# ZackAttack614/BlackBird

Hardware: AMD Instinct MI355X
Metric: selfplay_games_per_sec (higher is better)
Workload: dtype f32 (float32 operands split exactly into 3 bf16 values, 6 bf16 MFMA products each, f32 accumulate)

## Files before the change

### blackbird_amd/csrc/tree.hip.h

```cpp
#pragma once
#include "games.hip.h"
#include "rng.hip.h"
#include "starts.h"
#include "stamps.hip.h"

#define NODE_EXPANDED 1
#define NODE_TERMINAL 2
#define NODE_CACHED 4
#define LEAF_RECORDED 0x40000000
#define CHILD_NONE (-1)
#define CHILD_TERM_BIT 0x40000000

template <class G>
struct alignas(128) DenseNode {
    int32_t flags;
    uint32_t legal_mask;
    int32_t all;
    int32_t serial;
    double sq;
    double pad0;
    int32_t N[G::S];
    float Q[G::S];
    int32_t child[G::S];
    alignas(128) double cP[G::S];
    float W[G::S];
    typename G::State st;
};

struct ExampleHdr {
    uint32_t game_id;
    uint16_t ply;
    uint8_t player;
    int8_t z;
    uint32_t total;
    uint32_t n_children;
};

#define BB_SLOTS_TREE(B, Q, R)                                                                     \
    B(int32_t, root, 1) B(int32_t, root_N, 1) B(int32_t, n_nodes, 1) B(int32_t, ply, 1) B(int32_t, sims_left, 1)           \
    B(int32_t, pend_leaf, 1) B(int32_t, pend_expand, 1) B(int32_t, path_len, 1)                                            \
    B(int32_t, game_lid, 1)                                             \
    B(int32_t, sim_serial, 1) B(float, root_W, 1)                                                                          \
    B(int8_t, root_pp, 1)                                   \
    B(uint32_t, path, MP)                                                                \
        \
    R(int32_t, path_N, MP) R(int32_t, path_all, MP)       \
    R(float, path_W, MP)                                                               \
    Q(int32_t, leaf_flags, 1)
#define BB_SLOTS_ANC(X)                                                                                 \
       \
    X(uint32_t, anc, ANC)                                                                                                   \
    X(int32_t, anc_len, 1) X(int32_t, top_N, 1)
#define BB_SLOTS_MAILBOX(B, Q)                                                 \
    B(uint32_t, leaf_game_id, 1) B(int32_t, leaf_serial, 1) B(float, eval_value, 1) Q(float, eval_policy, PS)              \
    B(uint64_t, evals, 1)                                                              \
    B(uint64_t, ctr, 8)
#define BB_SLOTS_OUT(X)                                                       \
    X(int32_t, out_action, 1) X(int32_t, out_root_plays, 1) X(int32_t, out_child_plays, S)                                 \
    X(float, out_root_winrate, 1) X(float, out_child_value, S)
#define BB_SLOTS_RESUME(X) X(int32_t, resume_cur, 1) X(int32_t, resume_depth, 1)
#define BB_SLOTS_POST(X) X(int, post_slot, 1)
#define BB_ROW_NONE(...)
#define BB_SLOT_ARRAYS(X) BB_SLOTS_TREE(X, X, X) BB_SLOTS_ANC(X) BB_SLOTS_MAILBOX(X, X) BB_SLOTS_OUT(X) BB_SLOTS_RESUME(X) BB_SLOTS_POST(X)
#define BB_SLOT_SHADOWED(X) BB_SLOTS_TREE(X, BB_ROW_NONE, BB_ROW_NONE) BB_SLOTS_MAILBOX(X, BB_ROW_NONE)
#define BB_SLOT_POINTER(T, f, per) T *f;
#define BB_SHADOW_MEMBER(T, f, per) T f[GW * (per)];
#define BB_SHADOW_LOAD(o, f, per) for (int i = threadIdx.x; i < n * (per); i += nthreads) f[i] = o.f[(size_t)g0 * (per) + i];
#define BB_SHADOW_STORE(o, f, per) for (int i = threadIdx.x; i < n * (per); i += nthreads) o.f[(size_t)g0 * (per) + i] = f[i];

struct TreeDev {
    int n_slots, node_cap, sims_per_move, max_plies, kind, max_depth, evaluator, priors_ones;
    int salt_per_game, max_games;
    int gpw;
    double c_puct;
    uint64_t seed, salt;
    uint32_t first_game_id;
    BB_SLOTS_TREE(BB_SLOT_POINTER, BB_SLOT_POINTER, BB_SLOT_POINTER)
    int track_anc;
    BB_SLOTS_ANC(BB_SLOT_POINTER)
    void *leaf_state;
    BB_SLOTS_MAILBOX(BB_SLOT_POINTER, BB_SLOT_POINTER)
    void *nodes;
    int n_games_target;
    double temp;
    uint8_t *examples;
    int32_t *game_hdr;
    int example_bytes;
    BB_SLOTS_OUT(BB_SLOT_POINTER)
    const double *in_u;
    BB_SLOTS_RESUME(BB_SLOT_POINTER)
    int *post_count;
    BB_SLOTS_POST(BB_SLOT_POINTER)
    int level_budget;
    int slot_offset;
    int lid_stride;
    int pool_g0;
    int *visit_pool;
    float noise_alpha;
    void *eval_cache;
    int eval_cache_log2;
    unsigned long long *eval_cache_ctr;
    unsigned long long *stamps;
    const void *starts;
    int n_starts;
    double temp_late;
    int temp_plies;
};

template <int STEP>
__device__ __forceinline__ int dpp_step_i(int v) {
    if (STEP == 0) return __builtin_amdgcn_update_dpp(v, v, 0xB1, 0xf, 0xf, false);
    if (STEP == 1) return __builtin_amdgcn_update_dpp(v, v, 0x4E, 0xf, 0xf, false);
    if (STEP == 2) return __builtin_amdgcn_update_dpp(v, v, 0x141, 0xf, 0xf, false);
    return __builtin_amdgcn_update_dpp(v, v, 0x140, 0xf, 0xf, false);
}
template <int STEP>
__device__ __forceinline__ double dpp_step_d(double v) {
    long long b = __double_as_longlong(v);
    int lo = dpp_step_i<STEP>((int)(b & 0xffffffffll)), hi = dpp_step_i<STEP>((int)(b >> 32));
    return __longlong_as_double(((long long)hi << 32) | (unsigned int)lo);
}

template <int S>
__device__ __forceinline__ int grp_sum_i(int v) {
    v += dpp_step_i<0>(v);
    v += dpp_step_i<1>(v);
    v += dpp_step_i<2>(v);
    if (S == 16) v += dpp_step_i<3>(v);
    return v;
}

template <int A, int S>
__device__ __forceinline__ double grp_np_sum(double x) {
    double a[A];
#pragma unroll
    for (int k = 0; k < A; k++) a[k] = __shfl(x, k, S);
    if (A < 8) {
        double res = 0.;
#pragma unroll
        for (int k = 0; k < A; k++) res += a[k];
        return res;
    } else {
        double r[8];
#pragma unroll
        for (int j = 0; j < 8; j++) r[j] = a[j];
        int i = 8;
        for (; i < A - (A % 8); i += 8)
            for (int j = 0; j < 8; j++) r[j] += a[i + j];
        double res = ((r[0] + r[1]) + (r[2] + r[3])) + ((r[4] + r[5]) + (r[6] + r[7]));
        for (; i < A; i++) res += a[i];
        return res;
    }
}

template <int S, int STEP>
__device__ __forceinline__ void argmax_step(double &u, int &idx, int &payload) {
    double ou = dpp_step_d<STEP>(u);
    int oi = dpp_step_i<STEP>(idx), op = dpp_step_i<STEP>(payload);
    if (ou > u || (ou == u && oi < idx)) {
        u = ou;
        idx = oi;
        payload = op;
    }
}
template <int S>
__device__ __forceinline__ int grp_argmax(double u, int idx, int &payload) {
    (void)idx;
    double m = u;
    m = __builtin_fmax(m, dpp_step_d<0>(m));
    m = __builtin_fmax(m, dpp_step_d<1>(m));
    m = __builtin_fmax(m, dpp_step_d<2>(m));
    if (S == 16) m = __builtin_fmax(m, dpp_step_d<3>(m));
    const unsigned long long eq = __ballot(u == m);
    const int l64 = (int)__lane_id();
    const unsigned grp = (unsigned)(eq >> (l64 & ~(S - 1))) & ((1u << S) - 1u);
    const int win = __ffs(grp) - 1;
    payload = __shfl(payload, win, S);
    return win;
}

__device__ __forceinline__ double puct_score(double q, double cPi, double sq, int Ni, bool legal) {
    double u = q + __ddiv_rn(cPi * sq, 1.0 + (double)Ni);
    return legal ? u : -1.0;
}
#ifndef BB_PUCT_FILTER
#define BB_PUCT_FILTER 1
#endif
template <int S>
__device__ __forceinline__ int grp_argmax_puct(float qf, double cPi, double sq, int Ni, bool legal, int &payload) {
#if BB_PUCT_FILTER
    const float num = (float)(cPi * sq);
    const float uf = legal ? __builtin_fmaf(num, __builtin_amdgcn_rcpf((float)(Ni + 1)), qf) : -1.0f;
    float mf = uf;
    mf = __builtin_fmaxf(mf, __int_as_float(dpp_step_i<0>(__float_as_int(mf))));
    mf = __builtin_fmaxf(mf, __int_as_float(dpp_step_i<1>(__float_as_int(mf))));
    mf = __builtin_fmaxf(mf, __int_as_float(dpp_step_i<2>(__float_as_int(mf))));
    if (S == 16) mf = __builtin_fmaxf(mf, __int_as_float(dpp_step_i<3>(__float_as_int(mf))));
    const bool mine = uf >= mf - mf * 0x1p-18f && uf >= 0.0f;
    const unsigned long long cand = __ballot(mine);
    const int l64 = (int)__lane_id();
    const unsigned grp = (unsigned)(cand >> (l64 & ~(S - 1))) & ((1u << S) - 1u);
    if (__ballot((grp & (grp - 1u)) != 0u || grp == 0u) == 0ull) {
        const int win = __ffs(grp) - 1;
        int p = mine ? payload : 0;
        p |= dpp_step_i<0>(p);
        p |= dpp_step_i<1>(p);
        p |= dpp_step_i<2>(p);
        if (S == 16) p |= dpp_step_i<3>(p);
        payload = p;
        return win;
    }
#endif
    return grp_argmax<S>(puct_score((double)qf, cPi, sq, Ni, legal), 0, payload);
}
__device__ __forceinline__ double child_q(const TreeDev &d, float Qi, float Wi, int Ni) {
    if (d.evaluator != 2) return (double)Qi;
    return Ni > 0 ? (double)Wi / (double)Ni : 0.0;
}

__device__ __forceinline__ uint32_t path_word(int node, int player, int a) {
    return ((uint32_t)node << 6) | ((uint32_t)player << 4) | (uint32_t)a;
}
#define ANC_BROKEN (-1)

template <class G, bool REC = false>
__device__ __forceinline__ void backup_path(const TreeDev &d, int g, int lane, DenseNode<G> *pool, int plen, float v01,
                                            int prev) {
    constexpr int S = G::S;
    const float vflip = 1.0f - v01;
    const size_t p0 = (size_t)g * G::MAXPATH;
    auto edge = [&](uint32_t e, int k) __attribute__((always_inline)) {
        const int a = e & 15, pl = (e >> 4) & 3;
        DenseNode<G> *pn = pool + (e >> 6);
        int n, all;
        float w;
        if constexpr (REC) { n = d.path_N[p0 + k]; all = d.path_all[p0 + k]; w = d.path_W[p0 + k]; }
        else { n = pn->N[a]; all = pn->all; w = pn->W[a]; }
        n += 1;
        all += 1;
        w += (pl == prev) ? v01 : vflip;
        pn->N[a] = n;
        pn->W[a] = w;
        pn->Q[a] = __fdiv_rn(w, (float)n);
        pn->all = all;
        pn->sq = __dsqrt_rn(1.0 + (double)all);
    };
    for (int k = lane; k < plen; k += S) edge(d.path[p0 + k], k);
    if constexpr (!REC) {
        if (d.track_anc) {
            const uint32_t *anc = d.anc + (size_t)g * (d.max_plies + 2);
            const int na = d.anc_len[g];
            for (int k = lane; k < na; k += S) edge(anc[k], 0);
            if (lane == 0) d.top_N[g] += 1;
        }
    }
    if (lane == 0) {
        d.root_N[g] += 1;
        int pp = d.root_pp[g];
        if (pp) d.root_W[g] += (pp == prev) ? v01 : vflip;
    }
}

template <class G, bool REC = false>
__device__ __forceinline__ void phase_apply(const TreeDev &d, int g, int lane) {
    using Node = DenseNode<G>;
    constexpr int S = G::S, A = G::A;
    const int leaf = d.pend_leaf[g];
    if (leaf < 0) return;
    int lf = 0;
    if constexpr (REC) lf = d.leaf_flags[g] & ~LEAF_RECORDED;
    Node *pool = (Node *)d.nodes + (size_t)(g + d.pool_g0) * d.node_cap;
    Node *node = pool + leaf;
    auto add_flag = [&](int bit) __attribute__((always_inline)) {
        if constexpr (REC) node->flags = lf | bit;
        else node->flags |= bit;
    };
    const typename G::State st = ((const typename G::State *)d.leaf_state)[g];
    const float v = d.eval_value[g];
    const int expand_rec = REC ? d.pend_expand[g] : 0;
    auto expand = [&]() __attribute__((always_inline)) { return REC ? expand_rec : d.pend_expand[g]; };
    if (expand()) {
        const uint32_t mask = G::legal_mask(st);
        double x = 0.0;
        if (lane < A) x = (double)d.eval_policy[(size_t)g * S + lane] * (double)((mask >> lane) & 1u);
        const double tot = grp_np_sum<A, S>(x);
        node->N[lane] = 0;
        node->Q[lane] = 0.f;
        node->W[lane] = 0.f;
        node->child[lane] = CHILD_NONE;
        node->cP[lane] = (lane < A) ? d.c_puct * __ddiv_rn(x, tot) : 0.0;
        if (lane == 0) {
            add_flag(NODE_EXPANDED);
            node->legal_mask = mask;
            node->all = 0;
            node->sq = 1.0;
        }
    }
    const int player = gs_player(st), prev = gs_prev(st);
    const bool f32_eval = REC || d.evaluator != 2;
    float v01 = v;
    if (f32_eval) {
        v01 = (v + 1.0f) * 0.5f;
        if (player != prev) v01 = 1.0f - v01;
    }
    if (f32_eval && !expand() && ((REC ? lf : node->flags) & NODE_TERMINAL) && lane == 0) {
        node->pad0 = (double)v01;
        add_flag(NODE_CACHED);
    }
    backup_path<G, REC>(d, g, lane, pool, d.path_len[g], v01, prev);
    if (lane == 0) d.pend_leaf[g] = -1;
}

template <class G>
__device__ __forceinline__ int create_child(const TreeDev &d, int g, DenseNode<G> *pool, DenseNode<G> *parent,
                                            const typename G::State &pst, int a, int lane, int &nn,
                                            typename G::State &st2, bool &terminal, int *flags_out = nullptr) {
    int idx = nn;
    st2 = pst;
    G::apply(st2, a);
    int w = G::winner(st2, a);
    terminal = w >= 0;
    if (idx >= d.node_cap) return CHILD_NONE;
    int word = idx | (terminal ? CHILD_TERM_BIT : 0);
    nn = idx + 1;
    const int cflags = (terminal ? (NODE_TERMINAL | ((w + 1) << 8)) : 0) | (gs_player(st2) << 4);
    if (flags_out) *flags_out = cflags;
    if (lane == 0) {
        DenseNode<G> *c = pool + idx;
        c->st = st2;
        c->flags = cflags;
        c->legal_mask = 0;
        c->all = 0;
        c->serial = idx;
        parent->child[a] = word;
        d.n_nodes[g] = idx + 1;
        d.ctr[(size_t)g * 8 + 2] += 1;
    }
    return word;
}

template <class G>
__device__ __forceinline__ uint32_t expand_ones(const TreeDev &d, DenseNode<G> *node, const typename G::State &st,
                                                int lane, double &cPi) {
    uint32_t mask = G::legal_mask(st);
    cPi = (lane < G::A && ((mask >> lane) & 1u)) ? d.c_puct * 1.0 : 0.0;
    node->N[lane] = 0;
    node->Q[lane] = 0.f;
    node->W[lane] = 0.f;
    node->child[lane] = CHILD_NONE;
    node->cP[lane] = cPi;
    if (lane == 0) {
        node->flags |= NODE_EXPANDED;
        node->legal_mask = mask;
        node->all = 0;
        node->sq = 1.0;
    }
    return mask;
}

template <class G>
__device__ __forceinline__ void post_leaf(const TreeDev &d, int g, int cur, const typename G::State &st, int flags_word, int expand,
                                          int depth) {
    ((typename G::State *)d.leaf_state)[g] = st;
    d.leaf_game_id[g] = d.first_game_id + (uint32_t)d.game_lid[g];
    d.leaf_serial[g] = cur;
    d.pend_leaf[g] = cur;
    if (d.leaf_flags) d.leaf_flags[g] = flags_word;
    d.pend_expand[g] = expand;
    d.path_len[g] = depth;
    d.sim_serial[g] += 1;
    d.evals[g] += 1;
}

template <class G>
__device__ void phase_select(const TreeDev &d, int g, int lane) {
    using Node = DenseNode<G>;
    constexpr int S = G::S, A = G::A;
    if (d.game_lid[g] < 0 || d.sims_left[g] <= 0) return;
    Node *pool = (Node *)d.nodes + (size_t)(g + d.pool_g0) * d.node_cap;
    uint32_t *path = d.path + (size_t)g * G::MAXPATH;
    int cur = d.root[g];
    int nn = d.n_nodes[g];
    int depth = 0, expand = 0, overflow = 0, term_leaf = 0;
    const bool inline_expand = d.priors_ones != 0;
    const bool fixed = d.kind == 1, rollout = d.evaluator == 2;
    typename G::State st;
    int flags = 0;
    bool have = false;
    IF_STAMPS(long long acc_load = 0, acc_iter = 0;)
    for (int it = 0;; it++) {
        IF_STAMPS(long long ts0 = clock64(); acc_iter++;)
        Node *node = pool + cur;
        typename G::State st_l = node->st;
        int flags_l = node->flags;
        uint32_t mask = node->legal_mask;
        double sq = node->sq;
        int Ni = node->N[lane];
        float Qi = node->Q[lane];
        float Wi = rollout ? node->W[lane] : 0.f;
        double cPi = node->cP[lane];
        int ci = node->child[lane];
        asm volatile("" ::"v"(flags_l), "v"(mask), "v"(sq), "v"(Ni), "v"(Qi), "v"(cPi), "v"(ci));
        IF_STAMPS(acc_load += clock64() - ts0;)
        if (!have) {
            st = st_l;
            flags = flags_l;
        }
        have = false;
        if (fixed && it >= d.max_depth) break;
        if (!(flags & NODE_EXPANDED)) {
            if (flags & NODE_TERMINAL) { term_leaf = 1; break; }
            if (!inline_expand) { expand = 1; break; }
            mask = expand_ones<G>(d, node, st, lane, cPi);
            if (!fixed) break;
            Ni = 0;
            Qi = 0.f;
            Wi = 0.f;
            sq = 1.0;
            ci = CHILD_NONE;
        }
        if (mask == 0) break;
        double u = puct_score(child_q(d, Qi, Wi, Ni), cPi, sq, Ni, lane < A && ((mask >> lane) & 1u));
        int child = ci;
        int a = grp_argmax<S>(u, lane, child);
        if (depth >= G::MAXPATH) { overflow = 1; break; }
        if (child == CHILD_NONE) {
            typename G::State st2;
            bool terminal;
            child = create_child<G>(d, g, pool, node, st, a, lane, nn, st2, terminal);
            if (child == CHILD_NONE) { overflow = 1; break; }
            if (lane == 0) path[depth] = path_word(cur, (flags >> 4) & 3, a);
            st = st2;
            flags = (terminal ? NODE_TERMINAL : 0) | (gs_player(st2) << 4);
            have = true;
        } else {
            if (lane == 0) path[depth] = path_word(cur, (flags >> 4) & 3, a);
        }
        depth++;
        cur = child & ~CHILD_TERM_BIT;
    }
    if (lane == 0) {
        IF_STAMPS(stamp_add(d.stamps, TS_ROW_LOAD, acc_load); stamp_add(d.stamps, TS_ITERATIONS, acc_iter); stamp_add(d.stamps, TS_DESCENTS, 1);)
        post_leaf<G>(d, g, cur, st, 0, expand, depth);
        d.sims_left[g] -= 1;
        uint64_t *c = d.ctr + (size_t)g * 8;
        c[0] += 1;
        c[1] += (uint64_t)depth;
        c[3] += (uint64_t)term_leaf;
        c[6] += (uint64_t)overflow;
    }
}

template <class G>
__global__ void __launch_bounds__(256) k_tree_step(TreeDev d) {
    constexpr int S = G::S;
    int t = blockIdx.x * blockDim.x + threadIdx.x;
    int wv = t >> 6, l64 = t & 63;
    if (l64 >= d.gpw * S) return;
    int g = wv * d.gpw + l64 / S, lane = l64 % S;
    if (g >= d.n_slots) return;
    const long long t0 = stamp_clock();
    phase_apply<G>(d, g, lane);
    const long long t1 = stamp_clock();
    __threadfence_block();
    const long long t2 = stamp_clock();
    phase_select<G>(d, g, lane);
    const long long t3 = stamp_clock();
    if ((threadIdx.x & 63) == 0) {
        stamp_add(d.stamps, TS_APPLY, t1 - t0);
        stamp_add(d.stamps, TS_FENCE, t2 - t1);
        stamp_add(d.stamps, TS_SELECT, t3 - t2);
        stamp_add(d.stamps, TS_WAVES, 1);
    }
}

template <class G>
__global__ void __launch_bounds__(256) k_tree_apply(TreeDev d) {
    constexpr int S = G::S;
    int t = blockIdx.x * blockDim.x + threadIdx.x;
    int g = t / S, lane = t % S;
    if (g >= d.n_slots) return;
    phase_apply<G>(d, g, lane);
}

template <class G>
__device__ __forceinline__ int choose_move(const TreeDev &d, int g, int lane, double temp, double u, int &total, int &Ni_out,
                           float &Wi_out) {
    using Node = DenseNode<G>;
    constexpr int S = G::S, A = G::A;
    Node *pool = (Node *)d.nodes + (size_t)(g + d.pool_g0) * d.node_cap;
    Node *node = pool + d.root[g];
    if (!(node->flags & NODE_EXPANDED)) {
        total = 0;
        Ni_out = 0;
        Wi_out = 0.f;
        return -3;
    }
    uint32_t mask = node->legal_mask;
    bool legal = lane < A && ((mask >> lane) & 1u);
    int Ni = legal ? node->N[lane] : 0;
    float Wi = legal ? node->W[lane] : 0.f;
    Ni_out = Ni;
    Wi_out = Wi;
    int all = grp_sum_i<S>(Ni);
    total = all;
    if (temp == 0.0) {
        double uu = puct_score(child_q(d, node->Q[lane], Wi, Ni), node->cP[lane], node->sq, Ni, legal);
        int dummy = 0;
        return grp_argmax<S>(uu, lane, dummy);
    }
    double it = 1.0 / temp;
    double w = (it == 1.0) ? (double)Ni : pow((double)Ni, it);
    double ws[A];
#pragma unroll
    for (int k = 0; k < A; k++) ws[k] = __shfl(w, k, S);
    double allp = 0.0;
#pragma unroll
    for (int k = 0; k < A; k++) allp += ws[k];
    if (!(allp > 0.0 && allp < INFINITY)) return -4;
    double last = 0.0;
#pragma unroll
    for (int k = 0; k < A; k++) last += __ddiv_rn(ws[k], allp);
    double run = 0.0;
    int act = A - 1;
    bool found = false;
#pragma unroll
    for (int k = 0; k < A; k++) {
        run += __ddiv_rn(ws[k], allp);
        if (!found && __ddiv_rn(run, last) > u) {
            act = k;
            found = true;
        }
    }
    return act;
}

template <class G>
__global__ void __launch_bounds__(256) k_sample(TreeDev d, double temp) {
    constexpr int S = G::S;
    int t = blockIdx.x * blockDim.x + threadIdx.x;
    int g = t / S, lane = t % S;
    if (g >= d.n_slots) return;
    if (d.game_lid[g] < 0) {
        if (lane == 0 && d.out_action) d.out_action[g] = -3;
        return;
    }
    double u = d.in_u ? d.in_u[g] : bb_u53(d.seed, d.first_game_id + (uint32_t)d.game_lid[g], (uint32_t)d.ply[g]);
    int total, Ni;
    float Wi;
    int act = choose_move<G>(d, g, lane, temp, u, total, Ni, Wi);
    if (d.out_child_plays) d.out_child_plays[(size_t)g * S + lane] = Ni;
    if (d.out_child_value) d.out_child_value[(size_t)g * S + lane] = Wi;
    if (lane == 0) {
        if (d.out_action) d.out_action[g] = act;
        if (d.out_root_plays) d.out_root_plays[g] = d.root_N[g];
        if (d.out_root_winrate) {
            int n = d.root_N[g];
            float w = d.root_W[g];
            d.out_root_winrate[g] = n > 0 ? ((d.evaluator == 2) ? (float)((double)w / (double)n) : __fdiv_rn(w, (float)n)) : 0.f;
        }
    }
}

template <class G, bool CHAIN = true>
__device__ __forceinline__ void advance_root(const TreeDev &d, int g, int lane, int a, typename G::State &new_st) {
    using Node = DenseNode<G>;
    Node *pool = (Node *)d.nodes + (size_t)(g + d.pool_g0) * d.node_cap;
    Node *node = pool + d.root[g];
    typename G::State st = node->st;
    if (!(node->flags & NODE_EXPANDED)) {
        new_st = st;
        G::apply(new_st, a);
        if (lane == 0) {
            Node *r = pool;
            r->st = new_st;
            r->flags = gs_player(new_st) << 4;
            r->serial = 0;
            d.n_nodes[g] = 1;
            d.root[g] = 0;
            d.root_N[g] = 0;
            d.root_W[g] = 0.f;
            d.root_pp[g] = 0;
            if (d.track_anc) {
                d.anc_len[g] = 0;
                d.top_N[g] = 0;
            }
        }
        return;
    }
    int child = node->child[a];
    int cn = node->N[a];
    float cw = node->W[a];
    if (child == CHILD_NONE) {
        bool terminal;
        int nn = d.n_nodes[g];
        child = create_child<G>(d, g, pool, node, st, a, lane, nn, new_st, terminal);
        if (child == CHILD_NONE) {
            child = 0;
            cn = 0;
            cw = 0.f;
            if (lane == 0) {
                pool->st = new_st;
                pool->flags = gs_player(new_st) << 4;
                d.n_nodes[g] = 1;
                d.ctr[(size_t)g * 8 + 6] += 1;
            }
        }
    } else {
        new_st = pool[child & ~CHILD_TERM_BIT].st;
    }
    if (lane == 0) {
        if (d.track_anc) {
            if (child == 0 && cn == 0 && d.n_nodes[g] == 1) {
                d.anc_len[g] = 0;
                d.top_N[g] = 0;
            } else if constexpr (!CHAIN) {
                if (d.anc_len[g] < d.max_plies + 2) {
                    d.anc[(size_t)g * (d.max_plies + 2) + d.anc_len[g]] = path_word(d.root[g], gs_player(st), a);
                    d.anc_len[g] += 1;
                }
            } else {
                const int na = d.anc_len[g], cap = d.max_plies + 2;
                if (na >= 0 && na < cap) {
                    d.anc[(size_t)g * cap + na] = path_word(d.root[g], gs_player(st), a);
                    d.anc_len[g] = na + 1;
                } else {
                    d.anc_len[g] = ANC_BROKEN;
                }
            }
        }
        d.root[g] = child & ~CHILD_TERM_BIT;
        d.root_N[g] = cn;
        d.root_W[g] = cw;
        d.root_pp[g] = (int8_t)gs_player(st);
    }
}

template <class G>
__global__ void __launch_bounds__(256) k_reset_roots(TreeDev d) {
    int g = blockIdx.x * blockDim.x + threadIdx.x;
    if (g >= d.n_slots || !d.track_anc || d.game_lid[g] < 0 || d.anc_len[g] <= 0) return;
    {
        const int na = d.anc_len[g];
        const bool parked = d.resume_cur[g] >= 0, posted = d.pend_leaf[g] >= 0;
        const int plen = parked ? d.resume_depth[g] : d.path_len[g];
        if (parked || posted) {
            if (plen + na <= G::MAXPATH) {
                uint32_t *path = d.path + (size_t)g * G::MAXPATH;
                const uint32_t *anc = d.anc + (size_t)g * (d.max_plies + 2);
                for (int k = plen - 1; k >= 0; k--) path[k + na] = path[k];
                for (int k = 0; k < na; k++) path[k] = anc[k];
                if (parked) d.resume_depth[g] = plen + na;
                else d.path_len[g] = plen + na;
            } else {
                d.ctr[(size_t)g * 8 + 6] += 1;
            }
        }
    }
    d.root[g] = (int)(d.anc[(size_t)g * (d.max_plies + 2)] >> 6);
    d.root_N[g] = d.top_N[g];
    d.root_W[g] = 0.f;
    d.root_pp[g] = 0;
    d.anc_len[g] = 0;
}

template <class G>
__global__ void __launch_bounds__(64) k_node_view(TreeDev d, int g, int node, int32_t *child_out, int32_t *plays_out, float *value_out,
                                                   typename G::State *state_out, int32_t *info_out) {
    using Node = DenseNode<G>;
    const int lane = threadIdx.x;
    if (lane >= G::S) return;
    Node *pool = (Node *)d.nodes + (size_t)(g + d.pool_g0) * d.node_cap;
    if (node < 0) node = d.root[g];
    const Node *n = pool + node;
    const bool exp = (n->flags & NODE_EXPANDED) != 0;
    child_out[lane] = exp ? n->child[lane] : CHILD_NONE;
    plays_out[lane] = exp ? n->N[lane] : 0;
    value_out[lane] = exp ? n->W[lane] : 0.f;
    if (lane == 0) {
        *state_out = n->st;
        info_out[0] = n->flags;
        info_out[1] = (int32_t)(exp ? n->legal_mask : 0u);
        info_out[2] = node;
    }
}

template <class G>
__global__ void __launch_bounds__(256) k_move_roots(TreeDev d, const int32_t *actions) {
    constexpr int S = G::S;
    int t = blockIdx.x * blockDim.x + threadIdx.x;
    int g = t / S, lane = t % S;
    if (g >= d.n_slots) return;
    int a = actions[g];
    if (a < 0 || a >= G::A || d.game_lid[g] < 0) return;
    typename G::State ns;
    advance_root<G>(d, g, lane, a, ns);
    if (lane == 0) d.ply[g] += 1;
}

template <class G>
__device__ __forceinline__ void reset_slot(const TreeDev &d, int g, int lid, const typename G::State &st) {
    using Node = DenseNode<G>;
    Node *pool = (Node *)d.nodes + (size_t)(g + d.pool_g0) * d.node_cap;
    pool->st = st;
    pool->flags = gs_player(st) << 4;
    pool->legal_mask = 0;
    pool->all = 0;
    pool->serial = 0;
    d.n_nodes[g] = 1;
    d.root[g] = 0;
    d.root_N[g] = 0;
    d.root_W[g] = 0.f;
    d.root_pp[g] = 0;
    d.ply[g] = 0;
    d.pend_leaf[g] = -1;
    d.pend_expand[g] = 0;
    d.path_len[g] = 0;
    d.sim_serial[g] = 0;
    d.game_lid[g] = lid;
    if (d.leaf_flags) d.leaf_flags[g] = 0;
    if (d.track_anc) {
        d.anc_len[g] = 0;
        d.top_N[g] = 0;
    }
}

template <class G>
__global__ void __launch_bounds__(256) k_set_roots(TreeDev d, int n, const int32_t *slots,
                                                   const typename G::State *states, const uint32_t *game_ids) {
    int i = blockIdx.x * blockDim.x + threadIdx.x;
    if (i >= n) return;
    int g = slots ? slots[i] : i;
    if (g < 0 || g >= d.n_slots) return;
    reset_slot<G>(d, g, game_ids ? (int)game_ids[i] : g, states[i]);
    d.sims_left[g] = 0;
}

__global__ void __launch_bounds__(256) k_add_sims(TreeDev d, int sims, const uint8_t *mask = nullptr) {
    int g = blockIdx.x * blockDim.x + threadIdx.x;
    if (g >= d.n_slots) return;
    if (d.game_lid[g] >= 0 && (!mask || mask[g])) d.sims_left[g] = sims;
}

template <class G>
__global__ void __launch_bounds__(256) k_get_roots(TreeDev d, typename G::State *out) {
    int g = blockIdx.x * blockDim.x + threadIdx.x;
    if (g >= d.n_slots) return;
    out[g] = ((DenseNode<G> *)d.nodes + (size_t)(g + d.pool_g0) * d.node_cap + d.root[g])->st;
}

template <class G>
__device__ __forceinline__ typename G::State start_state(const TreeDev &d, int lid) {
    const typename G::State *t = (const typename G::State *)d.starts;
    if (t && lid >= 0) return t[lid % d.n_starts];
    return G::initial();
}

template <class G>
__global__ void __launch_bounds__(256) k_check_starts(int n, const typename G::State *states, uint8_t *verdict) {
    int i = blockIdx.x * blockDim.x + threadIdx.x;
    if (i >= n) return;
    const typename G::State st = states[i];
    int v = BB_START_OK;
    if (G::winner(st, -1) >= 0) v = BB_START_FINISHED;
    else if (G::legal_mask(st) == 0) v = BB_START_NO_MOVE;
    verdict[i] = (uint8_t)v;
}

template <class G>
__global__ void __launch_bounds__(256) k_selfplay_begin(TreeDev d) {
    int g = blockIdx.x * blockDim.x + threadIdx.x;
    if (g >= d.n_slots) return;
    if (g + d.slot_offset < d.n_games_target) {
        reset_slot<G>(d, g, g + d.slot_offset, start_state<G>(d, g + d.slot_offset));
        d.sims_left[g] = d.sims_per_move;
    } else {
        reset_slot<G>(d, g, -1, start_state<G>(d, -1));
        d.sims_left[g] = 0;
    }
}

template <class G>
__device__ __forceinline__ uint8_t *example_ptr(const TreeDev &d, int lid, int ply) {
    return d.examples + ((size_t)lid * (d.max_plies + 1) + ply) * d.example_bytes;
}

template <class G>
__device__ __forceinline__ void write_example(const TreeDev &d, int lid, int ply, const typename G::State &st, int lane, int Ni,
                              int total, uint32_t gid) {
    uint8_t *p = example_ptr<G>(d, lid, ply);
    if (lane == 0) {
        ExampleHdr h;
        h.game_id = gid;
        h.ply = (uint16_t)ply;
        h.player = (uint8_t)gs_player(st);
        h.z = 0;
        h.total = (uint32_t)total;
        h.n_children = G::A;
        *(ExampleHdr *)p = h;
        *(typename G::State *)(p + sizeof(ExampleHdr)) = st;
    }
    ((uint32_t *)(p + sizeof(ExampleHdr) + sizeof(typename G::State)))[lane] = (uint32_t)Ni;
}

template <class G, bool CHAIN = true>
__device__ __forceinline__ void selfplay_move_body(const TreeDev &d, int g, int lane) {
    using Node = DenseNode<G>;
    constexpr int S = G::S;
    int lid = d.game_lid[g];
    if (lid < 0) return;
    Node *pool = (Node *)d.nodes + (size_t)(g + d.pool_g0) * d.node_cap;
    typename G::State st = pool[d.root[g]].st;
    uint32_t gid = d.first_game_id + (uint32_t)lid;
    int ply = d.ply[g];
    double u = bb_u53(d.seed, gid, (uint32_t)ply);
    int total, Ni;
    float Wi;
    int act = choose_move<G>(d, g, lane, ply < d.temp_plies ? d.temp : d.temp_late, u, total, Ni, Wi);
    if (act < 0) {
        if (lane == 0) {
            d.game_lid[g] = -1;
            d.ctr[(size_t)g * 8 + 6] += 1;
        }
        return;
    }
    write_example<G>(d, lid, ply, st, lane, Ni, total, gid);
    typename G::State ns;
    advance_root<G, CHAIN>(d, g, lane, act, ns);
    __threadfence_block();
    ply += 1;
    int w = G::winner(ns, -1);
    bool over = w >= 0 || ply >= d.max_plies;
    if (!over) {
        if (lane == 0) {
            d.ply[g] = ply;
            d.sims_left[g] = d.sims_per_move;
            d.ctr[(size_t)g * 8 + 5] += 1;
        }
        return;
    }
    write_example<G>(d, lid, ply, ns, lane, 0, 0, gid);
    __threadfence_block();
    for (int k = lane; k <= ply; k += S) {
        ExampleHdr *h = (ExampleHdr *)example_ptr<G>(d, lid, k);
        h->z = (w <= 0) ? 0 : (h->player == w ? 1 : -1);
    }
    __threadfence();
    if (lane == 0) {
        int32_t *gh = d.game_hdr + (size_t)lid * 4;
        gh[0] = ply + 1;
        gh[1] = w;
        gh[2] = ply;
        __threadfence();
        gh[3] = 1;
        uint64_t *c = d.ctr + (size_t)g * 8;
        c[4] += 1;
        c[5] += 1;
        c[7] += (uint64_t)(ply + 1);
        int next = lid + d.lid_stride;
        if (next < d.n_games_target) {
            reset_slot<G>(d, g, next, start_state<G>(d, next));
            d.sims_left[g] = d.sims_per_move;
        } else {
            d.game_lid[g] = -1;
            d.sims_left[g] = 0;
        }
    }
}

template <class G>
__global__ void __launch_bounds__(256) k_selfplay_move(TreeDev d) {
    constexpr int S = G::S;
    int t = blockIdx.x * blockDim.x + threadIdx.x;
    int g = t / S, lane = t % S;
    if (g >= d.n_slots) return;
    phase_apply<G>(d, g, lane);
    __threadfence_block();
    selfplay_move_body<G>(d, g, lane);
}

struct NoPostHook {
    __device__ __forceinline__ void operator()(int, int) const {}
};
template <class G, bool REC = false, class OnPost = NoPostHook>
__device__ bool async_game(const TreeDev &d, int g, int lane, OnPost on_post = OnPost(), LevelStamps *light_out = nullptr) {
    using Node = DenseNode<G>;
    constexpr int S = G::S, A = G::A;
    if (d.game_lid[g] < 0) return false;
    Node *pool = (Node *)d.nodes + (size_t)(g + d.pool_g0) * d.node_cap;
    LevelStamps light;
    if (d.pend_leaf[g] >= 0) {
        if (REC && (d.leaf_flags[g] & LEAF_RECORDED)) phase_apply<G, true>(d, g, lane);
        else phase_apply<G>(d, g, lane);
        if (lane == 0) d.sims_left[g] -= 1;
        __threadfence_block();
    }
    int budget = d.level_budget;
    uint32_t *path = d.path + (size_t)g * G::MAXPATH;
    int sims_done = 0, depth_sum = 0, term_hits = 0;
    bool posted = false;
    for (;;) {
        if (d.sims_left[g] <= 0) {
            selfplay_move_body<G, !REC>(d, g, lane);
            __threadfence_block();
            if (d.game_lid[g] < 0) break;
        }
        int cur = d.resume_cur[g], depth = 0;
        if (cur >= 0) depth = d.resume_depth[g];
        else cur = d.root[g];
        int nn = d.n_nodes[g];
        typename G::State st;
        int flags = 0;
        enum { F_PARKED = 2, F_LEAF = 4, F_TERM = 8, F_EXPAND = 16, F_OVERFLOW = 32 };
        int fl = 0;
        IF_STAMPS_LIGHT(int lt_e = (int)clock64();)
        for (;;) {
            if (budget <= 0) { fl |= F_PARKED; break; }
            budget--;
            IF_STAMPS_LIGHT(light.levels++; int lt_a = (int)clock64();)
            Node *node = pool + cur;
            typename G::State st_l = node->st;
            int flags_l = node->flags;
            uint32_t mask = node->legal_mask;
            double sq = node->sq;
            int Ni = node->N[lane];
            float Qi = node->Q[lane];
            double cPi = node->cP[lane];
            int ci = node->child[lane];
            double cached = node->pad0;
            float Wi = 0.f;
            int all_l = 0;
            if (REC) {
                Wi = node->W[lane];
                all_l = node->all;
            }
            asm volatile("" ::"v"(flags_l), "v"(mask), "v"(sq), "v"(Ni), "v"(Qi), "v"(cPi), "v"(ci));
            IF_STAMPS_LIGHT(int lt_b = (int)clock64(); light.row_load += lt_b - lt_a;)
            st = st_l;
            flags = flags_l;
            if (!(flags & NODE_EXPANDED)) {
                fl |= F_LEAF;
                if (flags & NODE_TERMINAL) {
                    fl |= F_TERM;
                    if (flags & NODE_CACHED) {
                        float v01 = (float)cached;
                        __threadfence_block();
                        backup_path<G, REC>(d, g, lane, pool, depth, v01, gs_prev(st));
                        if (lane == 0) d.sims_left[g] -= 1;
                        __threadfence_block();
                        sims_done++;
                        depth_sum += depth;
                        term_hits++;
                        fl &= ~F_LEAF;
                    }
                } else {
                    fl |= F_EXPAND;
                }
                break;
            }
            static_assert(G::MAXPATH >= G::H * G::W + 2, "a descent places at most H*W stones");
            int child = ci;
            int a = grp_argmax_puct<S>(Qi, cPi, sq, Ni, lane < A && ((mask >> lane) & 1u), child);
            IF_STAMPS_LIGHT(asm volatile("" ::"v"(a), "v"(child)); light.puct += (int)clock64() - lt_b;)
            if (lane == 0) path[depth] = path_word(cur, (flags >> 4) & 3, a);
            if (REC) {
                if (lane == 0) d.path_all[(size_t)g * G::MAXPATH + depth] = all_l;
                if (lane == a) {
                    d.path_N[(size_t)g * G::MAXPATH + depth] = Ni;
                    d.path_W[(size_t)g * G::MAXPATH + depth] = Wi;
                }
            }
            if (child == CHILD_NONE) {
                typename G::State st2;
                bool terminal;
                child = create_child<G>(d, g, pool, node, st, a, lane, nn, st2, terminal, &flags);
                if (child == CHILD_NONE) { fl |= F_OVERFLOW | F_LEAF; break; }
                st = st2;
                depth++;
                cur = child & ~CHILD_TERM_BIT;
                fl |= F_LEAF | (terminal ? F_TERM : F_EXPAND);
                break;
            }
            depth++;
            cur = child & ~CHILD_TERM_BIT;
        }
        IF_STAMPS_LIGHT(light.loop += (int)clock64() - lt_e;)
        if (lane == 0) {
            d.resume_cur[g] = (fl & F_PARKED) ? cur : -1;
            d.resume_depth[g] = (fl & F_PARKED) ? depth : 0;
        }
        if (fl & F_PARKED) break;
        if (!(fl & F_LEAF)) {
            if (lane == 0) d.sim_serial[g] += 1;
            continue;
        }
        if (lane == 0) {
            post_leaf<G>(d, g, cur, st, REC ? (flags | LEAF_RECORDED) : 0, (fl & F_EXPAND) ? 1 : 0, depth);
            d.ctr[(size_t)g * 8 + 6] += (uint64_t)((fl & F_OVERFLOW) ? 1 : 0);
        }
        on_post(g, lane);
        sims_done++;
        depth_sum += depth;
        term_hits += (fl & F_TERM) ? 1 : 0;
        posted = true;
        break;
    }
    if (light_out) *light_out = light;
    if (lane == 0 && sims_done) {
        uint64_t *c = d.ctr + (size_t)g * 8;
        c[0] += (uint64_t)sims_done;
        c[1] += (uint64_t)depth_sum;
        c[3] += (uint64_t)term_hits;
    }
    return posted;
}

template <class G>
__global__ void __launch_bounds__(256) k_tree_async(TreeDev d, int round) {
    constexpr int S = G::S;
    int t = blockIdx.x * blockDim.x + threadIdx.x;
    int wv = t >> 6, l64 = t & 63;
    int g = wv * d.gpw + l64 / S, lane = l64 % S;
    bool live = l64 < d.gpw * S && g < d.n_slots;
    LevelStamps light;
    bool posted = live ? async_game<G>(d, g, lane, NoPostHook(), &light) : false;
    level_stamps_flush(d.stamps, light, live && lane == 0, l64);
    unsigned long long m = __ballot(posted && lane == 0);
    if (t == 0) d.post_count[(round + 2) & 3] = 0;
    if (m) {
        int leader = __ffsll((long long)m) - 1;
        int base = 0;
        if (l64 == leader) base = atomicAdd(&d.post_count[round & 3], __popcll(m));
        base = __shfl(base, leader, 64);
        if (posted && lane == 0) d.post_slot[base + __popcll(m & ((1ull << l64) - 1ull))] = g;
    }
}
```

Before: 9362.

## Prefetch next node row during recorded MCTS descent and hoist child creation

In the recorded (REC) descent path, the per-lane row for the next node is loaded right after the PUCT argmax, through global address-space pointers, so the load latency overlaps the path bookkeeping stores instead of stalling the next iteration. Child creation is moved out of the descent loop into a post-loop block, which shrinks the loop body. The cached terminal value is read only when it is needed. This adds live registers and one speculative extra row load when the chosen child does not exist yet. Whether the REC path is the one that runs during selfplay depends on the template instantiation.

```diff
diff --git a/blackbird_amd/csrc/tree.hip.h b/blackbird_amd/csrc/tree.hip.h
--- a/blackbird_amd/csrc/tree.hip.h
+++ b/blackbird_amd/csrc/tree.hip.h
@@ -879,6 +879,49 @@
     selfplay_move_body<G>(d, g, lane);
 }
 
+struct DescentRow {
+    int flags;
+    uint32_t mask;
+    int all;
+    double sq;
+    int N;
+    float Q;
+    int child;
+    double cP;
+    float W;
+};
+template <class G>
+__device__ __forceinline__ const __attribute__((address_space(1))) DenseNode<G> *descent_row_ptr(const DenseNode<G> *p) {
+    return (const __attribute__((address_space(1))) DenseNode<G> *)(const void *)p;
+}
+template <class G>
+__device__ __forceinline__ DescentRow descent_row(const DenseNode<G> *p, int lane) {
+    const auto *n = descent_row_ptr<G>(p);
+    DescentRow r;
+    r.flags = n->flags;
+    r.mask = n->legal_mask;
+    r.all = n->all;
+    r.sq = n->sq;
+    r.N = n->N[lane];
+    r.Q = n->Q[lane];
+    r.child = n->child[lane];
+    r.cP = n->cP[lane];
+    r.W = n->W[lane];
+    return r;
+}
+template <class G>
+__device__ __forceinline__ typename G::State descent_state(const DenseNode<G> *p) {
+    using State = typename G::State;
+    static_assert(sizeof(State) % 8 == 0 && __is_trivially_copyable(State), "a state is whole 64-bit words");
+    const auto *w = (const __attribute__((address_space(1))) uint64_t *)(const void *)&p->st;
+    uint64_t v[sizeof(State) / 8];
+#pragma unroll
+    for (size_t i = 0; i < sizeof(State) / 8; i++) v[i] = w[i];
+    State st;
+    __builtin_memcpy(&st, v, sizeof(State));
+    return st;
+}
+
 struct NoPostHook {
     __device__ __forceinline__ void operator()(int, int) const {}
 };
@@ -911,30 +954,39 @@
         int nn = d.n_nodes[g];
         typename G::State st;
         int flags = 0;
-        enum { F_PARKED = 2, F_LEAF = 4, F_TERM = 8, F_EXPAND = 16, F_OVERFLOW = 32 };
-        int fl = 0;
+        enum { F_PARKED = 2, F_LEAF = 4, F_TERM = 8, F_EXPAND = 16, F_OVERFLOW = 32, F_CREATE = 64 };
+        int fl = 0, act = 0;
         IF_STAMPS_LIGHT(int lt_e = (int)clock64();)
+        DescentRow nx = {};
+        if constexpr (REC) nx = descent_row<G>(pool + cur, lane);
         for (;;) {
             if (budget <= 0) { fl |= F_PARKED; break; }
             budget--;
             IF_STAMPS_LIGHT(light.levels++; int lt_a = (int)clock64();)
             Node *node = pool + cur;
-            typename G::State st_l = node->st;
-            int flags_l = node->flags;
-            uint32_t mask = node->legal_mask;
-            double sq = node->sq;
-            int Ni = node->N[lane];
-            float Qi = node->Q[lane];
-            double cPi = node->cP[lane];
-            int ci = node->child[lane];
-            double cached = node->pad0;
-            float Wi = 0.f;
+            typename G::State st_l;
+            int flags_l, Ni, ci;
+            uint32_t mask;
+            double sq, cPi, cached = 0.;
+            float Qi, Wi = 0.f;
             int all_l = 0;
-            if (REC) {
-                Wi = node->W[lane];
-                all_l = node->all;
+            if constexpr (REC) {
+                flags_l = nx.flags, mask = nx.mask, all_l = nx.all, sq = nx.sq, Ni = nx.N, Qi = nx.Q, ci = nx.child;
+                cPi = nx.cP, Wi = nx.W;
+                asm volatile("" ::"v"(flags_l), "v"(mask), "v"(all_l), "v"(sq), "v"(Ni), "v"(Qi), "v"(ci));
+                st_l = descent_state<G>(node);
+            } else {
+                st_l = node->st;
+                flags_l = node->flags;
+                mask = node->legal_mask;
+                sq = node->sq;
+                Ni = node->N[lane];
+                Qi = node->Q[lane];
+                cPi = node->cP[lane];
+                ci = node->child[lane];
+                cached = node->pad0;
+                asm volatile("" ::"v"(flags_l), "v"(mask), "v"(sq), "v"(Ni), "v"(Qi), "v"(cPi), "v"(ci));
             }
-            asm volatile("" ::"v"(flags_l), "v"(mask), "v"(sq), "v"(Ni), "v"(Qi), "v"(cPi), "v"(ci));
             IF_STAMPS_LIGHT(int lt_b = (int)clock64(); light.row_load += lt_b - lt_a;)
             st = st_l;
             flags = flags_l;
@@ -943,6 +995,7 @@
                 if (flags & NODE_TERMINAL) {
                     fl |= F_TERM;
                     if (flags & NODE_CACHED) {
+                        if constexpr (REC) cached = descent_row_ptr<G>(node)->pad0;
                         float v01 = (float)cached;
                         __threadfence_block();
                         backup_path<G, REC>(d, g, lane, pool, depth, v01, gs_prev(st));
@@ -961,6 +1014,11 @@
             static_assert(G::MAXPATH >= G::H * G::W + 2, "a descent places at most H*W stones");
             int child = ci;
             int a = grp_argmax_puct<S>(Qi, cPi, sq, Ni, lane < A && ((mask >> lane) & 1u), child);
+            if constexpr (REC) {
+                __builtin_amdgcn_sched_barrier(0);
+                nx = descent_row<G>(pool + (child == CHILD_NONE ? cur : (child & ~CHILD_TERM_BIT)), lane);
+                __builtin_amdgcn_sched_barrier(0);
+            }
             IF_STAMPS_LIGHT(asm volatile("" ::"v"(a), "v"(child)); light.puct += (int)clock64() - lt_b;)
             if (lane == 0) path[depth] = path_word(cur, (flags >> 4) & 3, a);
             if (REC) {
@@ -971,6 +1029,11 @@
                 }
             }
             if (child == CHILD_NONE) {
+                if constexpr (REC) {
+                    fl |= F_CREATE;
+                    act = a;
+                    break;
+                }
                 typename G::State st2;
                 bool terminal;
                 child = create_child<G>(d, g, pool, node, st, a, lane, nn, st2, terminal, &flags);
@@ -983,6 +1046,21 @@
             }
             depth++;
             cur = child & ~CHILD_TERM_BIT;
+        }
+        if constexpr (REC) {
+            if (fl & F_CREATE) {
+                typename G::State st2;
+                bool terminal;
+                const int child = create_child<G>(d, g, pool, pool + cur, st, act, lane, nn, st2, terminal, &flags);
+                if (child == CHILD_NONE) {
+                    fl |= F_OVERFLOW | F_LEAF;
+                } else {
+                    st = st2;
+                    depth++;
+                    cur = child & ~CHILD_TERM_BIT;
+                    fl |= F_LEAF | (terminal ? F_TERM : F_EXPAND);
+                }
+            }
         }
         IF_STAMPS_LIGHT(light.loop += (int)clock64() - lt_e;)
         if (lane == 0) {
```

After: 9981 (median of 6 runs). +6.6%, better.
